# taaha-khan/2023-CompaCT-Image-Compression

Hardware: AMD Instinct MI355X
Metric: MPixels/s encode+decode, 12-bit 512x512 CT batch, bytes-exact (higher is better)
Workload: dtype u16

## Files before the change

2023-compact-image-compression_amd/csrc/deflate_kernels.hip:

```cpp
#include <hip/hip_runtime.h>
#include <cstring>
#include <algorithm>

#include "cct_internal.h"
#include "../../include/compact_hip.h"

namespace cct {
namespace {

constexpr int MIN_MATCH = 3, MAX_MATCH = 258, WSIZE = 32768;
constexpr int MIN_LOOKAHEAD = MAX_MATCH + MIN_MATCH + 1;
constexpr int MAX_DIST = WSIZE - MIN_LOOKAHEAD;
constexpr int TOO_FAR = 4096;
constexpr int BLOCK_SYMS = 16383;
constexpr int BLOCK_SYMS_ML9 = 32767;
constexpr int L_CODES = 286, D_CODES = 30, BL_CODES = 19, HEAP_SIZE = 2 * L_CODES + 1;
constexpr int END_BLOCK = 256, MAX_BITS = 15, MAX_BL_BITS = 7;
constexpr uint32_t Z_FILTERED = 1, Z_HUFFMAN_ONLY = 2, Z_RLE = 3, Z_FIXED = 4;
__host__ __device__ __forceinline__ bool short_pass(uint32_t strategy) { return strategy == Z_HUFFMAN_ONLY || strategy == Z_RLE; }

__constant__ uint8_t c_extra_lbits[29] = {0,0,0,0,0,0,0,0,1,1,1,1,2,2,2,2,3,3,3,3,4,4,4,4,5,5,5,5,0};
__constant__ uint8_t c_extra_dbits[30] = {0,0,0,0,1,1,2,2,3,3,4,4,5,5,6,6,7,7,8,8,9,9,10,10,11,11,12,12,13,13};
__constant__ uint8_t c_extra_blbits[19] = {0,0,0,0,0,0,0,0,0,0,0,0,0,0,0,0,2,3,7};
__constant__ uint8_t c_bl_order[19] = {16,17,18,0,8,7,9,6,10,5,11,4,12,3,13,2,14,1,15};
// ... 1288 lines not shown
				if (R < 4) nlit_head = R;
				else if (R <= 6) { nlit_head = 1; tail_sym = 16u | ((R - 4u) << 5); }
				else {
					nlit_head = 1; nrep6 = 1 + (R - 7u) / 6u;
					const uint32_t r = (R - 7u) % 6u;
					if (r < 3) tail_lit = r; else tail_sym = 16u | ((r - 3u) << 5);
				}
			} else {
				nbig = R / 138u;
				const uint32_t r = R % 138u;
				if (r < 3) tail_lit = r;
				else if (r <= 10) tail_sym = 17u | ((r - 3u) << 5);
				else tail_sym = 18u | ((r - 11u) << 5);
			}
		}
		const uint32_t ntok = nlit_head + nrep6 + nbig + tail_lit + (tail_sym != 0xFFFFFFFFu ? 1u : 0u);
		uint32_t inc = ntok;
#pragma unroll
		for (int d = 1; d < 64; d <<= 1) { const uint32_t o = (uint32_t)__shfl_up((int)inc, d, 64); if (lane >= d) inc += o; }
		if (start) {
			uint32_t w = base + inc - ntok;
			for (uint32_t i = 0; i < nlit_head; i++) tk[w++] = (uint16_t)val;
			for (uint32_t i = 0; i < nrep6; i++) tk[w++] = (uint16_t)(16u | (3u << 5));
			for (uint32_t i = 0; i < nbig; i++) tk[w++] = (uint16_t)(18u | (127u << 5));
			for (uint32_t i = 0; i < tail_lit; i++) tk[w++] = (uint16_t)val;
			if (tail_sym != 0xFFFFFFFFu) tk[w++] = (uint16_t)tail_sym;
			if (nlit_head + tail_lit) atomicAdd(&S.hdr_bits[val], nlit_head + tail_lit);
			if (nrep6) atomicAdd(&S.hdr_bits[16], nrep6);
			if (nbig) atomicAdd(&S.hdr_bits[18], nbig);
			if (tail_sym != 0xFFFFFFFFu) atomicAdd(&S.hdr_bits[tail_sym & 31u], 1u);
		}
		base += (uint32_t)__shfl((int)inc, 63, 64);
	}
	if (lane == 0) S.ntok = (int)base;
}

__device__ __forceinline__ void hdr_or(TreeScratch &S, uint32_t pos, uint32_t value, uint32_t n)
{
	const uint32_t w = pos >> 5, sh = pos & 31u;
	atomicOr(&S.hdr_bits[w], value << sh);
	if (sh + n > 32u) atomicOr(&S.hdr_bits[w + 1], value >> (32u - sh));
}

__device__ void send_header(TreeScratch &S)
{
	const int lane = threadIdx.x;
	const int nbl = S.max_blindex + 1;
	if (lane == 0) hdr_or(S, 0, (uint32_t)(S.lmax + 1 - 257) | ((uint32_t)(S.dmax + 1 - 1) << 5) | ((uint32_t)(nbl - 4) << 10), 14);
	if (lane < nbl) hdr_or(S, 14u + 3u * (uint32_t)lane, S.blen[S.bl_order[lane]], 3);
	uint32_t base = 14u + 3u * (uint32_t)nbl;
	const uint16_t *tk = S.tok();
	const int nt = S.ntok;
	for (int c0 = 0; c0 < nt; c0 += 64) {
		const int i = c0 + lane;
		uint32_t nbits = 0, val = 0;
		if (i < nt) {
			const uint32_t sym = tk[i] & 31u, ex = tk[i] >> 5;
			const uint32_t cl = S.blen[sym];
			nbits = cl + S.extra_bl[sym];
			val = (uint32_t)S.bcode[sym] | (ex << cl);
		}
		uint32_t inc = nbits;
#pragma unroll
		for (int d = 1; d < 64; d <<= 1) { const uint32_t o = (uint32_t)__shfl_up((int)inc, d, 64); if (lane >= d) inc += o; }
		if (nbits) hdr_or(S, base + inc - nbits, val, nbits);
		base += (uint32_t)__shfl((int)inc, 63, 64);
	}
	if (lane == 0) S.hdr_nbits = base;
}

constexpr int TREE_BLOCKS = 1;

__device__ __forceinline__ uint32_t window_base(uint32_t top, uint32_t L, uint32_t strategy)
{
	const uint32_t lam = strategy == Z_HUFFMAN_ONLY ? 0u : strategy == Z_RLE ? (uint32_t)MAX_MATCH : (uint32_t)MIN_LOOKAHEAD - 1u;
	const uint32_t kf = L >= 65536u ? (L - 65536u) / 32768u + 1u : 0u;
	uint32_t k = 0;
	if (top >= 65536u - lam) k = min((top - (65536u - lam)) / 32768u + 1u, kf);
	if (k == kf && 32768u * k + (uint32_t)(WSIZE + MAX_DIST) <= top && L <= top + lam) k++;
	return 32768u * k;
}
__global__ void __launch_bounds__(64) dfl_tree_kernel(DeflateArgs a)
{
	__shared__ TreeScratch S4[TREE_BLOCKS];
	const int s = blockIdx.y, m0 = blockIdx.x * TREE_BLOCKS, lane = threadIdx.x;
	const uint32_t T = a.total_syms[s];
	const uint32_t L = a.in_sizes[s];
	const uint32_t BS = a.block_syms;
	uint32_t nfull = T / BS;
	if (T % BS == 0 && nfull > 0 && !short_pass(a.strategy) && a.postloop_lit[s]) nfull--;
	const uint32_t nblocks = nfull + 1;
	BlockMeta *meta = a.block_meta + (size_t)s * a.max_blocks;
	if ((uint32_t)m0 >= nblocks) return;
	const int nb = (int)min((uint32_t)TREE_BLOCKS, nblocks - (uint32_t)m0);
	const uint32_t *bend = a.blk_end + (size_t)s * a.max_blocks;
	const bool owner = lane < nb;
#ifdef CCT_TREE_PROF
	long long tp[16]; int tpi = 0;
#define TREE_STAMP() do { if (tpi < 16) tp[tpi++] = clock64(); } while (0)
#else
#define TREE_STAMP() do {} while (0)
#endif
	TREE_STAMP();

	for (int q = 0; q < nb; q++) {
		TreeScratch &S = S4[q];
		const int m = m0 + q;
		const bool last = (uint32_t)m == nblocks - 1;
		const uint32_t first = (uint32_t)m * BS;
		const uint32_t nsym = last ? T - first : BS;
		const uint32_t *sym = a.sym + (size_t)s * a.in_stride + first;
		for (int i = lane; i < HEAP_SIZE; i += 64) { S.freq[i] = 0; S.len[i] = 0; }
		for (int i = lane; i < L_CODES + 2; i += 64) S.code[i] = 0;
		for (int i = lane; i < 2 * D_CODES + 1; i += 64) { S.dfreq[i] = 0; S.dlen[i] = 0; S.ddad[i] = 0; }
		for (int i = lane; i < D_CODES + 2; i += 64) S.dcode[i] = 0;
		for (int i = lane; i < 2 * BL_CODES + 1; i += 64) { S.bfreq[i] = 0; S.blen[i] = 0; S.bdad[i] = 0; }
		for (int i = lane; i < BL_CODES + 1; i += 64) S.bcode[i] = 0;
		uint8_t *length_code = S.length_code(), *dist_code = S.dist_code();
		{
			uint8_t dc[8], lc4[4];
#pragma unroll
			for (int k = 0; k < 8; k++) dc[k] = c_dist_code[lane + 64 * k];
#pragma unroll
			for (int k = 0; k < 4; k++) lc4[k] = c_length_code[lane + 64 * k];
			const int l29 = min(lane, 28), l30 = min(lane, 29), l19 = min(lane, 18);
			const uint8_t xl = c_extra_lbits[l29], xd = c_extra_dbits[l30], xb = c_extra_blbits[l19], bo = c_bl_order[l19];
#pragma unroll
			for (int k = 0; k < 8; k++) dist_code[lane + 64 * k] = dc[k];
#pragma unroll
			for (int k = 0; k < 4; k++) length_code[lane + 64 * k] = lc4[k];
			if (lane < 29) S.extra_l[lane] = xl;
			if (lane < 30) S.extra_d[lane] = xd;
			if (lane < 19) { S.extra_bl[lane] = xb; S.bl_order[lane] = bo; }
		}
		uint32_t *hl = S.hist_l(), *hd = S.hist_d();
		for (int i = lane; i < L_CODES; i += 64) hl[i] = 0;
		if (lane < D_CODES) hd[lane] = 0;
		__syncthreads();
		{
			const uint32_t lasts = nsym ? nsym - 1 : 0;
			uint32_t nv[16];
#pragma unroll
			for (int k = 0; k < 16; k++) nv[k] = sym[min((uint32_t)(k * 64 + lane), lasts)];
			for (uint32_t i0 = 0; i0 < nsym; i0 += 64 * 16) {
				uint32_t v[16];
#pragma unroll
				for (int k = 0; k < 16; k++) v[k] = nv[k];
#pragma unroll
				for (int k = 0; k < 16; k++) nv[k] = sym[min(i0 + 1024u + (uint32_t)(k * 64 + lane), lasts)];
#pragma unroll
				for (int k = 0; k < 16; k++) {
					if (i0 + (uint32_t)(k * 64 + lane) >= nsym) continue;
					const uint32_t dist = v[k] >> 16, lc = v[k] & 0xFFu;
					if (dist == 0) atomicAdd(&hl[lc], 1u);
					else {
						const uint32_t d1 = dist - 1;
						atomicAdd(&hl[length_code[lc] + 256 + 1], 1u);
						atomicAdd(&hd[d1 < 256 ? dist_code[d1] : dist_code[256 + (d1 >> 7)]], 1u);
					}
				}
			}
		}
		__syncthreads();
		for (int i = lane; i < L_CODES; i += 64) S.freq[i] = (uint16_t)hl[i];
		if (lane < D_CODES) S.dfreq[lane] = (uint16_t)hd[lane];
		for (int i = lane; i < 160; i += 64) S.hdr_bits[i] = 0;
		if (lane == 0) { S.opt_len = 0; S.static_len = 0; S.hdr_nbits = 0; S.ntok = 0; S.btype = 0; S.max_blindex = 0; }
		__syncthreads();
		if (lane == 0) S.freq[END_BLOCK] = 1;
		for (int i = lane; i < HEAP_SIZE; i += 64) S.dad[i] = 0;
	}
	__syncthreads();
	TREE_STAMP();
#pragma unroll 1
	for (int kind = 0; kind < 3; kind++) {
		if (kind == 2) {
			if (owner) S4[lane].dyn_body_bits = S4[lane].opt_len;
			__syncthreads();
			for (int q = 0; q < nb; q++) {
				TreeScratch &S = S4[q];
				scan_tree_wave(S, view_of(S, 0), S.lmax);
				__syncthreads();
				scan_tree_wave(S, view_of(S, 1), S.dmax);
				__syncthreads();
				if (lane < BL_CODES) { S.bfreq[lane] = (uint16_t)S.hdr_bits[lane]; S.hdr_bits[lane] = 0; }
			}
			__syncthreads();
		}
		for (int q = 0; q < nb; q++) tree_leaves(S4[q], kind);
		__syncthreads();
		TREE_STAMP();
		for (int q = 0; q < nb; q++) tree_heap(S4[q], kind);
		__syncthreads();
		TREE_STAMP();
		for (int q = 0; q < nb; q++) tree_depths(S4[q], kind);
		__syncthreads();
		if (owner) {
			tree_fix(S4[lane], kind);
			if (kind == 0) S4[lane].lmax = S4[lane].max_code; else if (kind == 1) S4[lane].dmax = S4[lane].max_code;
		}
		__syncthreads();
		for (int q = 0; q < nb; q++) tree_codes(S4[q], kind);
		__syncthreads();
		TREE_STAMP();
	}
	if (owner) {
		TreeScratch &S = S4[lane];
		const int m = m0 + lane;
		const bool last = (uint32_t)m == nblocks - 1;
		const uint32_t first = (uint32_t)m * BS;
		const uint32_t nsym = last ? T - first : BS;
		const uint32_t in_begin = m == 0 ? 0u : bend[m - 1];
		const uint32_t in_end = last ? L : bend[m];
		int max_blindex;
		for (max_blindex = BL_CODES - 1; max_blindex >= 3; max_blindex--)
			if (S.blen[S.bl_order[max_blindex]] != 0) break;
		S.opt_len += 3 * ((uint32_t)max_blindex + 1) + 5 + 5 + 4;
		uint32_t opt_lenb = (S.opt_len + 3 + 7) >> 3;
		const uint32_t static_lenb = (S.static_len + 3 + 7) >> 3;
		if (static_lenb <= opt_lenb) opt_lenb = static_lenb;
		const uint32_t stored_len = in_end - in_begin;
		const bool in_window = in_begin >= window_base(last ? L : a.blk_top[(size_t)s * a.max_blocks + m], L, a.strategy);
		BlockMeta bm;
		bm.in_begin = in_begin; bm.stored_len = stored_len; bm.first_sym = first; bm.nsym = nsym; bm.last = last ? 1u : 0u;
		if (in_window && stored_len + 4 <= opt_lenb) {
			bm.type = 0; bm.hdr_nbits = 0; bm.body_bits = 0;
		} else if (a.strategy == Z_FIXED || static_lenb == opt_lenb) {
			bm.type = 1; bm.hdr_nbits = 0; bm.body_bits = S.static_len;
		} else {
			bm.type = 2; bm.hdr_nbits = 0;
			bm.body_bits = S.dyn_body_bits;
		}
		S.btype = (int)bm.type; S.max_blindex = max_blindex;
		meta[m] = bm;
		if (m == 0) a.n_blocks[s] = nblocks;
	}
	__syncthreads();
	for (int q = 0; q < nb; q++) {
		TreeScratch &S = S4[q];
		if (S.btype != 2) continue;
		send_header(S);
		__syncthreads();
		BlockTables *bt = a.block_tables + ((size_t)s * a.max_blocks + m0 + q);
		for (int i = lane; i * 32 < (int)S.hdr_nbits; i += 64) bt->hdr_bits[i] = S.hdr_bits[i];
		if (lane == 0) meta[m0 + q].hdr_nbits = S.hdr_nbits;
	}
	__syncthreads();
	TREE_STAMP();
#ifdef CCT_TREE_PROF
	if (s == 0 && m0 == 0 && lane == 0) {
		printf("[tree prof] nb=%d:", nb);
		for (int i = 1; i < tpi; i++) printf(" %lld", tp[i] - tp[i - 1]);
		printf("  (hist | leaves0 heap0 rest0 | scan+leaves1 heap1 rest1 | scan_tree+leaves2 heap2 rest2 | final)\n");
	}
#endif
	for (int q = 0; q < nb; q++) {
		TreeScratch &S = S4[q];
		BlockTables *bt = a.block_tables + ((size_t)s * a.max_blocks + m0 + q);
		for (int i = lane; i < L_CODES; i += 64) { bt->lcode[i] = S.code[i]; bt->llen[i] = (uint8_t)S.len[i]; }
		if (lane < D_CODES) { bt->dcode[lane] = S.dcode[lane]; bt->dlen[lane] = (uint8_t)S.dlen[lane]; }
	}
}

__global__ void __launch_bounds__(256) dfl_adler_kernel(DeflateArgs a)
{
	__shared__ unsigned long long sa[256], sb[256];
	const int s = blockIdx.x;
	const uint32_t L = a.in_sizes[s];
	const uint8_t *in = a.in + (size_t)s * a.in_stride;
	unsigned long long A = 0, B = 0;
	const uint32_t nfull = L / 16;
	constexpr int U = 8;
	for (uint32_t g0 = threadIdx.x; g0 < nfull; g0 += blockDim.x * U) {
		uint4 v[U];
#pragma unroll
		for (int u = 0; u < U; u++) v[u] = *reinterpret_cast<const uint4 *>(in + (size_t)min(g0 + (uint32_t)u * blockDim.x, nfull - 1) * 16);
#pragma unroll
		for (int u = 0; u < U; u++) {
			const uint32_t g = g0 + (uint32_t)u * blockDim.x;
			if (g >= nfull) continue;
			const uint32_t w[4] = {v[u].x, v[u].y, v[u].z, v[u].w};
			uint32_t sd = 0, sk = 0;
#pragma unroll
			for (int k = 0; k < 16; k++) { const uint32_t d = (w[k >> 2] >> ((k & 3) * 8)) & 0xFFu; sd += d; sk += (uint32_t)k * d; }
			A += sd;
			B += (unsigned long long)(L - g * 16) * sd - sk;
		}
	}
	if (threadIdx.x == 0)
		for (uint32_t i = nfull * 16; i < L; i++) { const unsigned long long d = in[i]; A += d; B += (unsigned long long)(L - i) * d; }
	sa[threadIdx.x] = A; sb[threadIdx.x] = B;
	__syncthreads();
	for (int st = 128; st > 0; st >>= 1) {
		if ((int)threadIdx.x < st) { sa[threadIdx.x] += sa[threadIdx.x + st]; sb[threadIdx.x] += sb[threadIdx.x + st]; }
		__syncthreads();
	}
	if (threadIdx.x == 0) {
		const uint32_t lo = (uint32_t)((1ull + sa[0]) % 65521ull);
		const uint32_t hi = (uint32_t)(((unsigned long long)L + sb[0]) % 65521ull);
		a.adler[s] = (hi << 16) | lo;
	}
}

__global__ void dfl_layout_kernel(DeflateArgs a, int n)
{
	const int s = blockIdx.x * blockDim.x + threadIdx.x;
	if (s >= n) return;
	uint8_t *out = a.out + (size_t)s * a.out_stride;
	for (int i = 0; i < 13; i++) out[i] = a.header13[i];
	out[13] = 0x78; out[14] = (uint8_t)a.zlib_flg;
	uint64_t bit = 8ull * 15;
	BlockMeta *meta = a.block_meta + (size_t)s * a.max_blocks;
	const uint32_t nb = a.n_blocks[s];
	for (uint32_t m = 0; m < nb; m++) {
		BlockMeta bm = meta[m];
		bm.bit_off = bit;
		if (bm.type == 0) {
			bit = (bit + 3 + 7) & ~7ull;
			bit += 32 + 8ull * bm.stored_len;
		} else {
			bit += 3 + bm.hdr_nbits + bm.body_bits;
		}
		if (bm.last) bit = (bit + 7) & ~7ull;
		meta[m] = bm;
	}
	const uint64_t byte = bit >> 3;
	const uint32_t ad = a.adler[s];
	out[byte + 0] = (uint8_t)(ad >> 24); out[byte + 1] = (uint8_t)(ad >> 16);
	out[byte + 2] = (uint8_t)(ad >> 8);  out[byte + 3] = (uint8_t)ad;
	a.out_sizes[s] = (uint32_t)(byte + 4);
}

__device__ __forceinline__ void or_bits(uint32_t *words, uint64_t bit, uint64_t value, int nbits)
{
	if (nbits == 0) return;
	const uint64_t w = bit >> 5;
	const int sh = (int)(bit & 31);
	const uint64_t lo = value << sh;
	const uint64_t hi = sh ? (value >> (64 - sh)) : 0ull;
	atomicOr(&words[w], (uint32_t)lo);
	if (sh + nbits > 32) atomicOr(&words[w + 1], (uint32_t)(lo >> 32));
	if (sh + nbits > 64) atomicOr(&words[w + 2], (uint32_t)hi);
}

__global__ void __launch_bounds__(256) dfl_emit_kernel(DeflateArgs a)
{
	__shared__ uint32_t wsum[4];
	__shared__ unsigned long long s_run;
	const int s = blockIdx.y, m = blockIdx.x;
	if ((uint32_t)m >= a.n_blocks[s]) return;
	const BlockMeta bm = a.block_meta[(size_t)s * a.max_blocks + m];
	const BlockTables *bt = a.block_tables + ((size_t)s * a.max_blocks + m);
	uint8_t *out = a.out + (size_t)s * a.out_stride;
	uint32_t *words = reinterpret_cast<uint32_t *>(out);
	const uint8_t *in = a.in + (size_t)s * a.in_stride;
	uint64_t bit = bm.bit_off;
	if (bm.type == 0) {
		if (threadIdx.x == 0) or_bits(words, bit, (uint64_t)bm.last, 3);
		const uint64_t byte = ((bit + 3 + 7) & ~7ull) >> 3;
		if (threadIdx.x == 0) {
			out[byte] = (uint8_t)(bm.stored_len & 0xFF); out[byte + 1] = (uint8_t)(bm.stored_len >> 8);
			out[byte + 2] = (uint8_t)(~bm.stored_len & 0xFF); out[byte + 3] = (uint8_t)((~bm.stored_len >> 8) & 0xFF);
		}
		for (uint32_t i = threadIdx.x; i < bm.stored_len; i += blockDim.x) out[byte + 4 + i] = in[bm.in_begin + i];
		return;
	}
	if (threadIdx.x == 0) or_bits(words, bit, (uint64_t)((bm.type << 1) + bm.last), 3);
	bit += 3;
	if (bm.type == 2) {
		for (uint32_t i = threadIdx.x; i * 32 < bm.hdr_nbits; i += blockDim.x) {
			const int nb = (int)min(32u, bm.hdr_nbits - i * 32);
			or_bits(words, bit + 32ull * i, bt->hdr_bits[i], nb);
		}
		bit += bm.hdr_nbits;
	}
	const uint32_t *sym = a.sym + (size_t)s * a.in_stride + bm.first_sym;
	const bool dyn = bm.type == 2;
	const int lane = threadIdx.x & 63, wave = threadIdx.x >> 6;
	__shared__ uint16_t t_lcode[L_CODES + 2], t_dcode[D_CODES + 2];
	__shared__ uint8_t t_llen[L_CODES + 2], t_dlen[D_CODES + 2];
	__shared__ uint32_t wbuf[400];
	__shared__ uint8_t t_length_code[256], t_dist_code[512], t_extra_l[32], t_extra_d[32];
	__shared__ uint16_t t_base_length[32], t_base_dist[32];
	{
		const int t = threadIdx.x, t2 = min(t + 256, L_CODES - 1), td = min(t, D_CODES - 1), t29 = min(t, 28), t30 = min(t, 29);
		const uint16_t *lsrc = dyn ? bt->lcode : c_static_lcode, *dsrc = dyn ? bt->dcode : c_static_dcode;
		const uint8_t *llsrc = dyn ? bt->llen : c_static_llen;
		const uint16_t lc0 = lsrc[t], lc1 = lsrc[t2];
		const uint8_t ll0 = llsrc[t], ll1 = llsrc[t2];
		const uint16_t dc = dsrc[td];
		uint8_t dl = bt->dlen[td];
		if (!dyn) dl = 5;
		const uint8_t k0 = c_dist_code[t], k1 = c_dist_code[t + 256], lcd = c_length_code[t];
		const uint8_t xl = c_extra_lbits[t29], xd = c_extra_dbits[t30];
		const uint16_t bl = c_base_length[t29], bd = c_base_dist[t30];
		t_lcode[t] = lc0; t_llen[t] = ll0;
		if (t + 256 < L_CODES) { t_lcode[t + 256] = lc1; t_llen[t + 256] = ll1; }
		if (t < D_CODES) { t_dcode[t] = dc; t_dlen[t] = dl; }
		t_dist_code[t] = k0; t_dist_code[t + 256] = k1; t_length_code[t] = lcd;
		if (t < 29) { t_extra_l[t] = xl; t_base_length[t] = bl; }
		if (t < 30) { t_extra_d[t] = xd; t_base_dist[t] = bd; }
	}
	if (threadIdx.x == 0) s_run = bit;
	for (int i = threadIdx.x; i < 400; i += blockDim.x) wbuf[i] = 0;
	__syncthreads();
	const uint32_t last_sym = bm.nsym ? bm.nsym - 1 : 0;
	uint32_t vnext = sym[min((uint32_t)threadIdx.x, last_sym)];
	for (uint32_t base = 0; base <= bm.nsym; base += blockDim.x) {
		const uint32_t i = base + threadIdx.x;
		uint64_t bits = 0;
		int nb = 0;
		const uint32_t v = vnext;
		vnext = sym[min(i + blockDim.x, last_sym)];
		if (i < bm.nsym) {
			uint32_t dist = v >> 16;
			const uint32_t lc = v & 0xFFu;
			if (dist == 0) {
				bits = t_lcode[lc];
				nb = t_llen[lc];
			} else {
				int code = t_length_code[lc];
				const int lsym = code + 256 + 1;
				bits = t_lcode[lsym];
				nb = t_llen[lsym];
				int extra = t_extra_l[code];
				if (extra) { bits |= (uint64_t)(lc - t_base_length[code]) << nb; nb += extra; }
				dist--;
				code = dist < 256 ? t_dist_code[dist] : t_dist_code[256 + (dist >> 7)];
				bits |= (uint64_t)t_dcode[code] << nb;
				nb += t_dlen[code];
				extra = t_extra_d[code];
				if (extra) { bits |= (uint64_t)(dist - t_base_dist[code]) << nb; nb += extra; }
			}
		} else if (i == bm.nsym) {
			bits = t_lcode[END_BLOCK];
			nb = t_llen[END_BLOCK];
		}
		uint32_t inc = (uint32_t)nb;
#pragma unroll
		for (int d = 1; d < 64; d <<= 1) {
			const uint32_t t = __shfl_up(inc, d);
			if (lane >= d) inc += t;
		}
		if (lane == 63) wsum[wave] = inc;
		__syncthreads();
		uint32_t wb = 0, tot = 0;
		for (int w = 0; w < 4; w++) { if (w < wave) wb += wsum[w]; tot += wsum[w]; }
		const uint64_t run = s_run;
		const uint32_t lbit = (uint32_t)(run & 31) + wb + inc - (uint32_t)nb;
		if (nb) {
			const uint32_t w0 = lbit >> 5, sh = lbit & 31;
			const uint64_t lo = bits << sh;
			atomicOr(&wbuf[w0], (uint32_t)lo);
			if (sh + nb > 32) atomicOr(&wbuf[w0 + 1], (uint32_t)(lo >> 32));
			if (sh + nb > 64) atomicOr(&wbuf[w0 + 2], (uint32_t)(bits >> (64 - sh)));
		}
		__syncthreads();
		const uint32_t nwords = ((uint32_t)(run & 31) + tot + 31) >> 5;
		const uint64_t gw = run >> 5;
		for (uint32_t k = threadIdx.x; k < nwords; k += blockDim.x) {
			const uint32_t v = wbuf[k];
			if (v) atomicOr(&words[gw + k], v);
			wbuf[k] = 0;
		}
		if (threadIdx.x == 0) s_run = run + tot;
		__syncthreads();
	}
}

__global__ void __launch_bounds__(256) dfl_pack_offsets_kernel(const uint32_t *sizes, int n, uint64_t *offsets, int exact)
{
	if (threadIdx.x == 0 && blockIdx.x == 0) {
		uint64_t acc = 0;
		for (int i = 0; i < n; i++) { offsets[i] = acc; acc += exact ? sizes[i] : ((sizes[i] + 15u) & ~15u); }
		offsets[n] = acc;
	}
}
__global__ void __launch_bounds__(256) dfl_pack_kernel(const uint8_t *src, size_t stride, const uint32_t *sizes,
                                                       const uint64_t *offsets, uint8_t *dst)
{
	const int s = blockIdx.y;
	const uint32_t n16 = (sizes[s] + 15u) >> 4;
	const uint4 *in = reinterpret_cast<const uint4 *>(src + (size_t)s * stride);
	uint4 *out = reinterpret_cast<uint4 *>(dst + offsets[s]);
	for (uint32_t i = blockIdx.x * blockDim.x + threadIdx.x; i < n16; i += gridDim.x * blockDim.x) out[i] = in[i];
}

__global__ void dfl_offsets2_kernel(DeflateArgs a, int n)
{
	const size_t per = a.in_stride / 64;
	for (size_t i = blockIdx.x * (size_t)blockDim.x + threadIdx.x; i < (size_t)n * per; i += (size_t)gridDim.x * blockDim.x)
		a.blk_entry[i] = 0xFFFFFFFFu;
}

__global__ void dfl_offsets_kernel(DeflateArgs a, int n)
{
	if (blockIdx.x == 0) {
		for (int s = threadIdx.x; s < n; s += blockDim.x) { a.postloop_lit[s] = 0; a.heavy_count[s] = 0; a.deep_count[s] = 0; a.run_end_count[s] = 0; }
		if (threadIdx.x == 0) *a.gen = *a.gen % GEN_MAX + 1u;
	}
	const size_t nrc = (size_t)n * 2 * (size_t)a.run_chunks;
	for (size_t t = (size_t)blockIdx.x * blockDim.x + threadIdx.x; t < nrc; t += (size_t)gridDim.x * blockDim.x) a.run_counts[t] = 0;
}

}

bool deflate_level_args(int level, DeflateArgs &a)
{
	static const uint32_t T[6][5] = {
		{4, 4, 16, 16, 0x5E}, {8, 16, 32, 32, 0x5E}, {8, 16, 128, 128, 0x9C},
		{8, 32, 128, 256, 0xDA}, {32, 128, 258, 1024, 0xDA}, {32, 258, 258, 4096, 0xDA},
	};
	if (level < 4 || level > 9) return false;
	const uint32_t *t = T[level - 4];
	a.good = t[0]; a.max_lazy = t[1]; a.nice = t[2]; a.max_chain = t[3]; a.zlib_flg = t[4];
	return true;
}

bool deflate_strategy_args(int level, int strategy, DeflateArgs &a)
{
	if (strategy < 0 || strategy > (int)Z_FIXED) return false;
	a.strategy = (uint32_t)strategy;
	a.min_len = strategy == (int)Z_FILTERED ? 6u : (uint32_t)MIN_MATCH;
	if (short_pass((uint32_t)strategy)) {
		if (level < 1 || level > 9) return false;
		a.good = a.max_lazy = a.nice = a.max_chain = 0;
		a.zlib_flg = 0x01;
		return true;
	}
	if (!deflate_level_args(level, a)) return false;
	if (strategy == (int)Z_FIXED) a.zlib_flg = 0x01;
	return true;
}

bool deflate_mem_level_args(int mem_level, DeflateArgs &a)
{
	if (mem_level != 8 && mem_level != 9) return false;
	a.hash_bits = (uint32_t)mem_level + 7u;
	a.block_syms = (1u << (mem_level + 6)) - 1u;
	return true;
}

hipError_t deflate_init_tables()
{
	uint8_t length_code[256]; uint16_t base_length[29]; uint8_t dist_code[512]; uint16_t base_dist[30];
	uint16_t static_lcode[288]; uint8_t static_llen[288]; uint16_t static_dcode[30];
	static const int xl[29] = {0,0,0,0,0,0,0,0,1,1,1,1,2,2,2,2,3,3,3,3,4,4,4,4,5,5,5,5,0};
	static const int xd[30] = {0,0,0,0,1,1,2,2,3,3,4,4,5,5,6,6,7,7,8,8,9,9,10,10,11,11,12,12,13,13};
	int length = 0, code, n, dist = 0;
	for (code = 0; code < 28; code++) {
		base_length[code] = (uint16_t)length;
		for (n = 0; n < (1 << xl[code]); n++) length_code[length++] = (uint8_t)code;
	}
	length_code[length - 1] = (uint8_t)code;
	base_length[28] = 0;
	for (code = 0; code < 16; code++) {
		base_dist[code] = (uint16_t)dist;
		for (n = 0; n < (1 << xd[code]); n++) dist_code[dist++] = (uint8_t)code;
	}
	dist >>= 7;
	for (; code < 30; code++) {
		base_dist[code] = (uint16_t)(dist << 7);
		for (n = 0; n < (1 << (xd[code] - 7)); n++) dist_code[256 + dist++] = (uint8_t)code;
	}
	uint16_t bl_count[16] = {0}, next_code[16];
	n = 0;
	while (n <= 143) { static_llen[n++] = 8; bl_count[8]++; }
	while (n <= 255) { static_llen[n++] = 9; bl_count[9]++; }
	while (n <= 279) { static_llen[n++] = 7; bl_count[7]++; }
	while (n <= 287) { static_llen[n++] = 8; bl_count[8]++; }
	unsigned c = 0;
	for (int bits = 1; bits <= 15; bits++) { c = (c + bl_count[bits - 1]) << 1; next_code[bits] = (uint16_t)c; }
	auto rev = [](unsigned v, int len) { unsigned r = 0; do { r |= v & 1; v >>= 1; r <<= 1; } while (--len > 0); return r >> 1; };
	for (n = 0; n < 288; n++) static_lcode[n] = (uint16_t)rev(next_code[static_llen[n]]++, static_llen[n]);
	for (n = 0; n < 30; n++) static_dcode[n] = (uint16_t)rev((unsigned)n, 5);
	hipError_t e;
	if ((e = hipMemcpyToSymbol(HIP_SYMBOL(c_length_code), length_code, sizeof length_code)) != hipSuccess) return e;
	if ((e = hipMemcpyToSymbol(HIP_SYMBOL(c_base_length), base_length, sizeof base_length)) != hipSuccess) return e;
	if ((e = hipMemcpyToSymbol(HIP_SYMBOL(c_dist_code), dist_code, sizeof dist_code)) != hipSuccess) return e;
	if ((e = hipMemcpyToSymbol(HIP_SYMBOL(c_base_dist), base_dist, sizeof base_dist)) != hipSuccess) return e;
	if ((e = hipMemcpyToSymbol(HIP_SYMBOL(c_static_lcode), static_lcode, sizeof static_lcode)) != hipSuccess) return e;
	if ((e = hipMemcpyToSymbol(HIP_SYMBOL(c_static_llen), static_llen, sizeof static_llen)) != hipSuccess) return e;
	if ((e = hipMemcpyToSymbol(HIP_SYMBOL(c_static_dcode), static_dcode, sizeof static_dcode)) != hipSuccess) return e;
	return hipSuccess;
}

size_t deflate_sort_temp_bytes(size_t total, int n)
{
	(void)total; (void)n;
	return 0;
}

static hipError_t launch_deflate_short(const DeflateArgs &a, int n, hipStream_t st)
{
	const bool ml9 = a.block_syms == (uint32_t)BLOCK_SYMS_ML9;
	const int gx = (int)std::min<size_t>(64, (a.in_stride + 255) / 256);
	if (a.strategy == Z_RLE) {
		hipLaunchKernelGGL((dfl_run_len_kernel<false, 15>), dim3(gx, n), dim3(256), 0, st, a);
		hipLaunchKernelGGL(dfl_rle_rec_kernel, dim3(gx, n), dim3(256), 0, st, a);
		hipLaunchKernelGGL(dfl_offsets2_kernel, dim3(256), dim3(256), 0, st, a, n);
		hipLaunchKernelGGL(dfl_walk_kernel, dim3(n), dim3(WALK_T), 0, st, a, n);
		if (ml9) hipLaunchKernelGGL(dfl_symbols_kernel<BLOCK_SYMS_ML9>, dim3(gx, n), dim3(256), 0, st, a);
		else hipLaunchKernelGGL(dfl_symbols_kernel<BLOCK_SYMS>, dim3(gx, n), dim3(256), 0, st, a);
	} else {
		if (ml9) hipLaunchKernelGGL(dfl_huff_symbols_kernel<BLOCK_SYMS_ML9>, dim3(gx, n), dim3(256), 0, st, a);
		else hipLaunchKernelGGL(dfl_huff_symbols_kernel<BLOCK_SYMS>, dim3(gx, n), dim3(256), 0, st, a);
	}
	hipLaunchKernelGGL(dfl_adler_kernel, dim3(n), dim3(256), 0, st, a);
	hipLaunchKernelGGL(dfl_tree_kernel, dim3((a.max_blocks + TREE_BLOCKS - 1) / TREE_BLOCKS, n), dim3(64), 0, st, a);
	hipLaunchKernelGGL(dfl_layout_kernel, dim3((n + 63) / 64), dim3(64), 0, st, a, n);
	hipLaunchKernelGGL(dfl_emit_kernel, dim3(a.max_blocks, n), dim3(256), 0, st, a);
	return hipGetLastError();
}

hipError_t launch_deflate(const DeflateArgs &a, int n, void *sort_temp, size_t sort_temp_bytes, hipStream_t st, hipStream_t side,
                          const hipEvent_t *ev)
{
	hipError_t e;
	const bool ml9 = a.hash_bits == 16;
	if ((a.hash_bits != 15 && !ml9) || a.block_syms != (uint32_t)(ml9 ? BLOCK_SYMS_ML9 : BLOCK_SYMS)) return hipErrorInvalidValue;
	if (ml9 && a.pos_mask != 0xFFFFFFFFu) return hipErrorInvalidValue;
	if ((e = hipMemsetAsync(a.out, 0, (size_t)n * a.out_stride, st)) != hipSuccess) return e;
	if (short_pass(a.strategy)) return launch_deflate_short(a, n, st);
	if ((e = hipMemsetAsync(a.sort_hist, 0, (size_t)n * SORT_HIST * 4, st)) != hipSuccess) return e;
	hipLaunchKernelGGL(dfl_offsets_kernel, dim3(64), dim3(256), 0, st, a, n);
	const int gx = (int)std::min<size_t>(64, (a.in_stride + 255) / 256);
	(void)sort_temp; (void)sort_temp_bytes;
	if (ml9) {
		hipLaunchKernelGGL((dfl_run_len_kernel<true, 16>), dim3(gx, n), dim3(256), 0, st, a);
		hipLaunchKernelGGL((dfl_sort_pass_kernel<true, 16>), dim3(n), dim3(1024), 0, st, a);
		hipLaunchKernelGGL((dfl_sort_pass_kernel<false, 16>), dim3(n), dim3(1024), 0, st, a);
	} else {
		hipLaunchKernelGGL((dfl_run_len_kernel<true, 15>), dim3(gx, n), dim3(256), 0, st, a);
		hipLaunchKernelGGL((dfl_sort_pass_kernel<true, 15>), dim3(n), dim3(1024), 0, st, a);
		hipLaunchKernelGGL((dfl_sort_pass_kernel<false, 15>), dim3(n), dim3(1024), 0, st, a);
	}
	const bool fork = side != nullptr && ev != nullptr;
	hipStream_t s2 = fork ? side : st;
	if (fork) {
		if ((e = hipEventRecord(ev[0], st)) != hipSuccess) return e;
		if ((e = hipStreamWaitEvent(s2, ev[0], 0)) != hipSuccess) return e;
	}
	hipLaunchKernelGGL(dfl_run_lists_kernel, dim3(a.run_chunks, n), dim3(256), 0, s2, a);
	hipLaunchKernelGGL(dfl_run_info_kernel, dim3(8, n), dim3(256), 0, s2, a);
	const int gm_cap = a.pos_mask == COMPACT_POS_MASK ? 256 : 2048;
	const int gm = (int)std::min<size_t>(gm_cap, (a.in_stride + 255) / 256), n8 = (n + 7) & ~7;
	if (a.max_chain < 16 || a.max_chain > 4096 || a.nice < 16 || a.nice > (uint32_t)MAX_MATCH) return hipErrorInvalidValue;
	const bool ql = (a.max_chain >> 2) <= (uint32_t)LIGHT_STEPS;
	if (a.pos_mask == COMPACT_POS_MASK) {
		if (ql) hipLaunchKernelGGL((dfl_match_kernel<true, true>), dim3(gm, n8), dim3(256), 0, st, a, n);
		else hipLaunchKernelGGL((dfl_match_kernel<true, false>), dim3(gm, n8), dim3(256), 0, st, a, n);
	} else if (a.pos_mask == 0xFFFFFFFFu) {
		if (ql) hipLaunchKernelGGL((dfl_match_kernel<false, true>), dim3(gm, n8), dim3(256), 0, st, a, n);
		else hipLaunchKernelGGL((dfl_match_kernel<false, false>), dim3(gm, n8), dim3(256), 0, st, a, n);
	} else return hipErrorInvalidValue;
	if (fork) {
		if ((e = hipEventRecord(ev[1], st)) != hipSuccess) return e;
		if ((e = hipEventRecord(ev[2], s2)) != hipSuccess) return e;
		if ((e = hipStreamWaitEvent(s2, ev[1], 0)) != hipSuccess) return e;
		if ((e = hipStreamWaitEvent(st, ev[2], 0)) != hipSuccess) return e;
	}
	hipLaunchKernelGGL(dfl_match_heavy_kernel, dim3(gx, n8), dim3(256), 0, s2, a, n);
	hipLaunchKernelGGL(dfl_adler_kernel, dim3(n), dim3(256), 0, s2, a);
	hipLaunchKernelGGL(dfl_match_run_kernel, dim3(gx, n8), dim3(256), 0, st, a, n);
	if (fork) {
		if ((e = hipEventRecord(ev[3], s2)) != hipSuccess) return e;
		if ((e = hipStreamWaitEvent(st, ev[3], 0)) != hipSuccess) return e;
	}
	hipLaunchKernelGGL(dfl_rec_kernel, dim3(gx, n), dim3(256), 0, st, a);
	hipLaunchKernelGGL(dfl_offsets2_kernel, dim3(256), dim3(256), 0, st, a, n);
	hipLaunchKernelGGL(dfl_walk_kernel, dim3(n), dim3(WALK_T), 0, st, a, n);
	if (ml9) hipLaunchKernelGGL(dfl_symbols_kernel<BLOCK_SYMS_ML9>, dim3(gx, n), dim3(256), 0, st, a);
	else hipLaunchKernelGGL(dfl_symbols_kernel<BLOCK_SYMS>, dim3(gx, n), dim3(256), 0, st, a);
	hipLaunchKernelGGL(dfl_tree_kernel, dim3((a.max_blocks + TREE_BLOCKS - 1) / TREE_BLOCKS, n), dim3(64), 0, st, a);
	hipLaunchKernelGGL(dfl_layout_kernel, dim3((n + 63) / 64), dim3(64), 0, st, a, n);
	hipLaunchKernelGGL(dfl_emit_kernel, dim3(a.max_blocks, n), dim3(256), 0, st, a);
	return hipGetLastError();
}

__global__ void __launch_bounds__(256) dfl_pack_exact_kernel(const uint8_t *src, size_t stride, const uint32_t *sizes,
                                                             const uint64_t *offsets, uint8_t *dst)
{
	const int s = blockIdx.y;
	const uint32_t nbytes = sizes[s];
	const uint8_t *in = src + (size_t)s * stride;
	uint8_t *out = dst + offsets[s];
	for (uint32_t i = blockIdx.x * blockDim.x + threadIdx.x; i < nbytes; i += gridDim.x * blockDim.x) out[i] = in[i];
}

hipError_t launch_pack(const uint8_t *src, size_t stride, const uint32_t *sizes, int n, uint64_t *offsets, uint8_t *dst,
                       int exact, hipStream_t st)
{
	hipLaunchKernelGGL(dfl_pack_offsets_kernel, dim3(1), dim3(64), 0, st, sizes, n, offsets, exact);
	if (exact) hipLaunchKernelGGL(dfl_pack_exact_kernel, dim3(32, n), dim3(256), 0, st, src, stride, sizes, offsets, dst);
	else hipLaunchKernelGGL(dfl_pack_kernel, dim3(16, n), dim3(256), 0, st, src, stride, sizes, offsets, dst);
	return hipGetLastError();
}

}
```

Before: 16100.

## Parallelize layout, pack offsets, multi-symbol emit, and replace memsets with bounded clears

The layout kernel now gives one wavefront per stream and passes block sizes between lanes with shuffles, and the pack-offsets kernel becomes a block-wide scan instead of a serial loop. The emit kernel now has each thread encode several symbols into local limbs, and double-buffers its shared word buffer so one barrier per iteration goes away. Its interior words are written with plain stores instead of atomics. Full-buffer memsets are replaced by a clear kernel that zeroes only the bounded output size, runs on the side stream, and also clears the sort histogram. The exact pack copy uses 32-bit words with shift alignment, and offsets2 is moved onto the side stream.

```diff
diff --git a/2023-compact-image-compression_amd/csrc/deflate_kernels.hip b/2023-compact-image-compression_amd/csrc/deflate_kernels.hip
--- a/2023-compact-image-compression_amd/csrc/deflate_kernels.hip
+++ b/2023-compact-image-compression_amd/csrc/deflate_kernels.hip
@@ -1614,33 +1614,38 @@
 	}
 }
 
-__global__ void dfl_layout_kernel(DeflateArgs a, int n)
-{
-	const int s = blockIdx.x * blockDim.x + threadIdx.x;
+__global__ void __launch_bounds__(64) dfl_layout_kernel(DeflateArgs a, int n)
+{
+	const int s = blockIdx.x, lane = threadIdx.x;
 	if (s >= n) return;
 	uint8_t *out = a.out + (size_t)s * a.out_stride;
-	for (int i = 0; i < 13; i++) out[i] = a.header13[i];
-	out[13] = 0x78; out[14] = (uint8_t)a.zlib_flg;
-	uint64_t bit = 8ull * 15;
 	BlockMeta *meta = a.block_meta + (size_t)s * a.max_blocks;
 	const uint32_t nb = a.n_blocks[s];
-	for (uint32_t m = 0; m < nb; m++) {
-		BlockMeta bm = meta[m];
-		bm.bit_off = bit;
-		if (bm.type == 0) {
-			bit = (bit + 3 + 7) & ~7ull;
-			bit += 32 + 8ull * bm.stored_len;
-		} else {
-			bit += 3 + bm.hdr_nbits + bm.body_bits;
-		}
-		if (bm.last) bit = (bit + 7) & ~7ull;
-		meta[m] = bm;
-	}
-	const uint64_t byte = bit >> 3;
 	const uint32_t ad = a.adler[s];
-	out[byte + 0] = (uint8_t)(ad >> 24); out[byte + 1] = (uint8_t)(ad >> 16);
-	out[byte + 2] = (uint8_t)(ad >> 8);  out[byte + 3] = (uint8_t)ad;
-	a.out_sizes[s] = (uint32_t)(byte + 4);
+	uint64_t bit = 8ull * 15;
+	for (uint32_t m0 = 0; m0 < nb; m0 += 64) {
+		const uint32_t m = m0 + (uint32_t)lane, cnt = min(64u, nb - m0);
+		const BlockMeta bm = meta[min(m, nb - 1)];
+		const uint32_t flags = (bm.type == 0 ? 1u : 0u) | (bm.last ? 2u : 0u);
+		const uint64_t size = bm.type == 0 ? 32 + 8ull * bm.stored_len : 3ull + bm.hdr_nbits + bm.body_bits;
+		uint64_t mine = 0;
+		for (uint32_t j = 0; j < cnt; j++) {
+			const uint32_t fj = __shfl(flags, (int)j);
+			const uint64_t zj = __shfl((unsigned long long)size, (int)j);
+			if (j == (uint32_t)lane) mine = bit;
+			bit = (fj & 1u) ? ((bit + 3 + 7) & ~7ull) + zj : bit + zj;
+			if (fj & 2u) bit = (bit + 7) & ~7ull;
+		}
+		if (m < nb) meta[m].bit_off = mine;
+	}
+	if (lane == 0) {
+		for (int i = 0; i < 13; i++) out[i] = a.header13[i];
+		out[13] = 0x78; out[14] = (uint8_t)a.zlib_flg;
+		const uint64_t byte = bit >> 3;
+		out[byte + 0] = (uint8_t)(ad >> 24); out[byte + 1] = (uint8_t)(ad >> 16);
+		out[byte + 2] = (uint8_t)(ad >> 8);  out[byte + 3] = (uint8_t)ad;
+		a.out_sizes[s] = (uint32_t)(byte + 4);
+	}
 }
 
 __device__ __forceinline__ void or_bits(uint32_t *words, uint64_t bit, uint64_t value, int nbits)
@@ -1655,10 +1660,16 @@
 	if (sh + nbits > 64) atomicOr(&words[w + 2], (uint32_t)hi);
 }
 
+#ifndef CCT_EMIT_K
+#define CCT_EMIT_K 4
+#endif
+constexpr int EMIT_K = CCT_EMIT_K;
+constexpr int EMIT_T = 256 * EMIT_K;
+constexpr int EMIT_LIMBS = (EMIT_K * 48 + 63) / 64;
+constexpr int EMIT_WBUF = EMIT_T * 48 / 32 + 8;
 __global__ void __launch_bounds__(256) dfl_emit_kernel(DeflateArgs a)
 {
-	__shared__ uint32_t wsum[4];
-	__shared__ unsigned long long s_run;
+	__shared__ uint32_t wsum[2][4];
 	const int s = blockIdx.y, m = blockIdx.x;
 	if ((uint32_t)m >= a.n_blocks[s]) return;
 	const BlockMeta bm = a.block_meta[(size_t)s * a.max_blocks + m];
@@ -1691,7 +1702,7 @@
 	const int lane = threadIdx.x & 63, wave = threadIdx.x >> 6;
 	__shared__ uint16_t t_lcode[L_CODES + 2], t_dcode[D_CODES + 2];
 	__shared__ uint8_t t_llen[L_CODES + 2], t_dlen[D_CODES + 2];
-	__shared__ uint32_t wbuf[400];
+	__shared__ uint32_t wbuf[2][EMIT_WBUF];
 	__shared__ uint8_t t_length_code[256], t_dist_code[512], t_extra_l[32], t_extra_d[32];
 	__shared__ uint16_t t_base_length[32], t_base_dist[32];
 	{
@@ -1713,80 +1724,122 @@
 		if (t < 29) { t_extra_l[t] = xl; t_base_length[t] = bl; }
 		if (t < 30) { t_extra_d[t] = xd; t_base_dist[t] = bd; }
 	}
-	if (threadIdx.x == 0) s_run = bit;
-	for (int i = threadIdx.x; i < 400; i += blockDim.x) wbuf[i] = 0;
+	for (int i = threadIdx.x; i < 2 * EMIT_WBUF; i += blockDim.x) (&wbuf[0][0])[i] = 0;
 	__syncthreads();
 	const uint32_t last_sym = bm.nsym ? bm.nsym - 1 : 0;
-	uint32_t vnext = sym[min((uint32_t)threadIdx.x, last_sym)];
-	for (uint32_t base = 0; base <= bm.nsym; base += blockDim.x) {
-		const uint32_t i = base + threadIdx.x;
-		uint64_t bits = 0;
-		int nb = 0;
-		const uint32_t v = vnext;
-		vnext = sym[min(i + blockDim.x, last_sym)];
-		if (i < bm.nsym) {
-			uint32_t dist = v >> 16;
-			const uint32_t lc = v & 0xFFu;
-			if (dist == 0) {
-				bits = t_lcode[lc];
-				nb = t_llen[lc];
-			} else {
-				int code = t_length_code[lc];
-				const int lsym = code + 256 + 1;
-				bits = t_lcode[lsym];
-				nb = t_llen[lsym];
-				int extra = t_extra_l[code];
-				if (extra) { bits |= (uint64_t)(lc - t_base_length[code]) << nb; nb += extra; }
-				dist--;
-				code = dist < 256 ? t_dist_code[dist] : t_dist_code[256 + (dist >> 7)];
-				bits |= (uint64_t)t_dcode[code] << nb;
-				nb += t_dlen[code];
-				extra = t_extra_d[code];
-				if (extra) { bits |= (uint64_t)(dist - t_base_dist[code]) << nb; nb += extra; }
-			}
-		} else if (i == bm.nsym) {
-			bits = t_lcode[END_BLOCK];
-			nb = t_llen[END_BLOCK];
-		}
-		uint32_t inc = (uint32_t)nb;
+	uint32_t vnext[EMIT_K];
+#pragma unroll
+	for (int k = 0; k < EMIT_K; k++) vnext[k] = sym[min((uint32_t)(threadIdx.x * EMIT_K + k), last_sym)];
+	uint64_t run = bit;
+	int par = 0;
+	for (uint32_t base = 0; base <= bm.nsym; base += EMIT_T, par ^= 1) {
+		const uint32_t i0 = base + threadIdx.x * EMIT_K;
+		uint32_t v[EMIT_K];
+#pragma unroll
+		for (int k = 0; k < EMIT_K; k++) v[k] = vnext[k];
+#pragma unroll
+		for (int k = 0; k < EMIT_K; k++) vnext[k] = sym[min(i0 + (uint32_t)(EMIT_T + k), last_sym)];
+		uint64_t acc[EMIT_LIMBS];
+#pragma unroll
+		for (int j = 0; j < EMIT_LIMBS; j++) acc[j] = 0;
+		uint32_t ltot = 0;
+#pragma unroll
+		for (int k = 0; k < EMIT_K; k++) {
+			const uint32_t i = i0 + k;
+			uint64_t bits = 0;
+			int nb = 0;
+			if (i < bm.nsym) {
+				uint32_t dist = v[k] >> 16;
+				const uint32_t lc = v[k] & 0xFFu;
+				if (dist == 0) {
+					bits = t_lcode[lc];
+					nb = t_llen[lc];
+				} else {
+					int code = t_length_code[lc];
+					const int lsym = code + 256 + 1;
+					bits = t_lcode[lsym];
+					nb = t_llen[lsym];
+					int extra = t_extra_l[code];
+					if (extra) { bits |= (uint64_t)(lc - t_base_length[code]) << nb; nb += extra; }
+					dist--;
+					code = dist < 256 ? t_dist_code[dist] : t_dist_code[256 + (dist >> 7)];
+					bits |= (uint64_t)t_dcode[code] << nb;
+					nb += t_dlen[code];
+					extra = t_extra_d[code];
+					if (extra) { bits |= (uint64_t)(dist - t_base_dist[code]) << nb; nb += extra; }
+				}
+			} else if (i == bm.nsym) {
+				bits = t_lcode[END_BLOCK];
+				nb = t_llen[END_BLOCK];
+			}
+			const uint32_t q = ltot >> 6, r = ltot & 63;
+			const uint64_t lo = bits << r, hi = r ? bits >> (64 - r) : 0ull;
+#pragma unroll
+			for (int j = 0; j < EMIT_LIMBS; j++) {
+				if (q == (uint32_t)j) acc[j] |= lo;
+				if (q + 1 == (uint32_t)j) acc[j] |= hi;
+			}
+			ltot += (uint32_t)nb;
+		}
+		uint32_t inc = ltot;
 #pragma unroll
 		for (int d = 1; d < 64; d <<= 1) {
 			const uint32_t t = __shfl_up(inc, d);
 			if (lane >= d) inc += t;
 		}
-		if (lane == 63) wsum[wave] = inc;
+		if (lane == 63) wsum[par][wave] = inc;
 		__syncthreads();
 		uint32_t wb = 0, tot = 0;
-		for (int w = 0; w < 4; w++) { if (w < wave) wb += wsum[w]; tot += wsum[w]; }
-		const uint64_t run = s_run;
-		const uint32_t lbit = (uint32_t)(run & 31) + wb + inc - (uint32_t)nb;
-		if (nb) {
-			const uint32_t w0 = lbit >> 5, sh = lbit & 31;
-			const uint64_t lo = bits << sh;
-			atomicOr(&wbuf[w0], (uint32_t)lo);
-			if (sh + nb > 32) atomicOr(&wbuf[w0 + 1], (uint32_t)(lo >> 32));
-			if (sh + nb > 64) atomicOr(&wbuf[w0 + 2], (uint32_t)(bits >> (64 - sh)));
+		for (int w = 0; w < 4; w++) { if (w < wave) wb += wsum[par][w]; tot += wsum[par][w]; }
+		uint32_t *wbf = wbuf[par];
+		const uint32_t lbit = (uint32_t)(run & 31) + wb + inc - ltot;
+		if (ltot) {
+			const uint32_t w0 = lbit >> 5, sh = lbit & 31, nw = (sh + ltot + 31) >> 5;
+#pragma unroll
+			for (int j = 0; j <= 2 * EMIT_LIMBS; j++) {
+				const uint32_t aj = j < 2 * EMIT_LIMBS ? (uint32_t)(acc[j >> 1] >> (32 * (j & 1))) : 0u;
+				const uint32_t ap = j > 0 ? (uint32_t)(acc[(j - 1) >> 1] >> (32 * ((j - 1) & 1))) : 0u;
+				const uint32_t w = (uint32_t)((((uint64_t)aj << 32) | ap) >> (32 - sh));
+				if ((uint32_t)j < nw && w) atomicOr(&wbf[w0 + j], w);
+			}
 		}
 		__syncthreads();
 		const uint32_t nwords = ((uint32_t)(run & 31) + tot + 31) >> 5;
 		const uint64_t gw = run >> 5;
 		for (uint32_t k = threadIdx.x; k < nwords; k += blockDim.x) {
-			const uint32_t v = wbuf[k];
-			if (v) atomicOr(&words[gw + k], v);
-			wbuf[k] = 0;
-		}
-		if (threadIdx.x == 0) s_run = run + tot;
+			const uint32_t w = wbf[k];
+			wbf[k] = 0;
+			if (k == 0 || k == nwords - 1) { if (w) atomicOr(&words[gw + k], w); }
+			else words[gw + k] = w;
+		}
+		run += tot;
+	}
+}
+
+__global__ void __launch_bounds__(256) dfl_pack_offsets_kernel(const uint32_t *sizes, int n, uint64_t *offsets, int exact)
+{
+	__shared__ unsigned long long wsum[4];
+	const int t = threadIdx.x, lane = t & 63, wave = t >> 6;
+	unsigned long long carry = 0;
+	for (int base = 0; base < n; base += 256) {
+		const int i = base + t;
+		const uint32_t sz = i < n ? sizes[i] : 0u;
+		const unsigned long long v = exact ? sz : (unsigned long long)((sz + 15u) & ~15u);
+		unsigned long long inc = v;
+#pragma unroll
+		for (int d = 1; d < 64; d <<= 1) {
+			const unsigned long long u = __shfl_up(inc, d);
+			if (lane >= d) inc += u;
+		}
+		if (lane == 63) wsum[wave] = inc;
 		__syncthreads();
-	}
-}
-
-__global__ void __launch_bounds__(256) dfl_pack_offsets_kernel(const uint32_t *sizes, int n, uint64_t *offsets, int exact)
-{
-	if (threadIdx.x == 0 && blockIdx.x == 0) {
-		uint64_t acc = 0;
-		for (int i = 0; i < n; i++) { offsets[i] = acc; acc += exact ? sizes[i] : ((sizes[i] + 15u) & ~15u); }
-		offsets[n] = acc;
-	}
+		unsigned long long wb = 0, tot = 0;
+		for (int w = 0; w < 4; w++) { if (w < wave) wb += wsum[w]; tot += wsum[w]; }
+		if (i < n) offsets[i] = carry + wb + inc - v;
+		carry += tot;
+		__syncthreads();
+	}
+	if (t == 0) offsets[n] = carry;
 }
 __global__ void __launch_bounds__(256) dfl_pack_kernel(const uint8_t *src, size_t stride, const uint32_t *sizes,
                                                        const uint64_t *offsets, uint8_t *dst)
@@ -1811,8 +1864,31 @@
 		for (int s = threadIdx.x; s < n; s += blockDim.x) { a.postloop_lit[s] = 0; a.heavy_count[s] = 0; a.deep_count[s] = 0; a.run_end_count[s] = 0; }
 		if (threadIdx.x == 0) *a.gen = *a.gen % GEN_MAX + 1u;
 	}
-	const size_t nrc = (size_t)n * 2 * (size_t)a.run_chunks;
-	for (size_t t = (size_t)blockIdx.x * blockDim.x + threadIdx.x; t < nrc; t += (size_t)gridDim.x * blockDim.x) a.run_counts[t] = 0;
+	const size_t nrc = (size_t)n * (SORT_HIST + 2 * (size_t)a.run_chunks);
+	for (size_t t = (size_t)blockIdx.x * blockDim.x + threadIdx.x; t < nrc; t += (size_t)gridDim.x * blockDim.x) a.sort_hist[t] = 0;
+}
+
+constexpr uint32_t CLEAR_SLACK = 64;
+__device__ __forceinline__ size_t clear_bytes(const DeflateArgs &a, int s)
+{
+	const size_t L = a.in_sizes[s];
+	const size_t bound = a.block_syms == (uint32_t)BLOCK_SYMS ? L + (L >> 12) + (L >> 14) + (L >> 25) + 13
+	                                                          : L + ((L + 7) >> 3) + ((L + 63) >> 6) + 5 + 6;
+	return min(a.out_stride, (13 + bound + CLEAR_SLACK + 15) & ~(size_t)15);
+}
+template <typename W>
+__global__ void __launch_bounds__(256) dfl_clear_kernel(DeflateArgs a)
+{
+	const int s = blockIdx.y;
+	const size_t units = clear_bytes(a, s) / sizeof(W);
+	W *out = reinterpret_cast<W *>(a.out + (size_t)s * a.out_stride);
+	W zero{};
+	for (size_t i = blockIdx.x * (size_t)blockDim.x + threadIdx.x; i < units; i += (size_t)gridDim.x * blockDim.x) out[i] = zero;
+}
+static void launch_clear(const DeflateArgs &a, int n, hipStream_t st)
+{
+	if (a.out_stride % 16 == 0 && (uintptr_t)a.out % 16 == 0) hipLaunchKernelGGL(dfl_clear_kernel<uint4>, dim3(16, n), dim3(256), 0, st, a);
+	else hipLaunchKernelGGL(dfl_clear_kernel<uint32_t>, dim3(32, n), dim3(256), 0, st, a);
 }
 
 }
@@ -1907,6 +1983,7 @@
 {
 	const bool ml9 = a.block_syms == (uint32_t)BLOCK_SYMS_ML9;
 	const int gx = (int)std::min<size_t>(64, (a.in_stride + 255) / 256);
+	launch_clear(a, n, st);
 	if (a.strategy == Z_RLE) {
 		hipLaunchKernelGGL((dfl_run_len_kernel<false, 15>), dim3(gx, n), dim3(256), 0, st, a);
 		hipLaunchKernelGGL(dfl_rle_rec_kernel, dim3(gx, n), dim3(256), 0, st, a);
@@ -1920,7 +1997,7 @@
 	}
 	hipLaunchKernelGGL(dfl_adler_kernel, dim3(n), dim3(256), 0, st, a);
 	hipLaunchKernelGGL(dfl_tree_kernel, dim3((a.max_blocks + TREE_BLOCKS - 1) / TREE_BLOCKS, n), dim3(64), 0, st, a);
-	hipLaunchKernelGGL(dfl_layout_kernel, dim3((n + 63) / 64), dim3(64), 0, st, a, n);
+	hipLaunchKernelGGL(dfl_layout_kernel, dim3(n), dim3(64), 0, st, a, n);
 	hipLaunchKernelGGL(dfl_emit_kernel, dim3(a.max_blocks, n), dim3(256), 0, st, a);
 	return hipGetLastError();
 }
@@ -1932,9 +2009,8 @@
 	const bool ml9 = a.hash_bits == 16;
 	if ((a.hash_bits != 15 && !ml9) || a.block_syms != (uint32_t)(ml9 ? BLOCK_SYMS_ML9 : BLOCK_SYMS)) return hipErrorInvalidValue;
 	if (ml9 && a.pos_mask != 0xFFFFFFFFu) return hipErrorInvalidValue;
-	if ((e = hipMemsetAsync(a.out, 0, (size_t)n * a.out_stride, st)) != hipSuccess) return e;
+	if ((a.out_stride & 3) || ((uintptr_t)a.out & 3)) return hipErrorInvalidValue;
 	if (short_pass(a.strategy)) return launch_deflate_short(a, n, st);
-	if ((e = hipMemsetAsync(a.sort_hist, 0, (size_t)n * SORT_HIST * 4, st)) != hipSuccess) return e;
 	hipLaunchKernelGGL(dfl_offsets_kernel, dim3(64), dim3(256), 0, st, a, n);
 	const int gx = (int)std::min<size_t>(64, (a.in_stride + 255) / 256);
 	(void)sort_temp; (void)sort_temp_bytes;
@@ -1955,6 +2031,8 @@
 	}
 	hipLaunchKernelGGL(dfl_run_lists_kernel, dim3(a.run_chunks, n), dim3(256), 0, s2, a);
 	hipLaunchKernelGGL(dfl_run_info_kernel, dim3(8, n), dim3(256), 0, s2, a);
+	launch_clear(a, n, s2);
+	hipLaunchKernelGGL(dfl_offsets2_kernel, dim3(256), dim3(256), 0, s2, a, n);
 	const int gm_cap = a.pos_mask == COMPACT_POS_MASK ? 256 : 2048;
 	const int gm = (int)std::min<size_t>(gm_cap, (a.in_stride + 255) / 256), n8 = (n + 7) & ~7;
 	if (a.max_chain < 16 || a.max_chain > 4096 || a.nice < 16 || a.nice > (uint32_t)MAX_MATCH) return hipErrorInvalidValue;
@@ -1980,12 +2058,11 @@
 		if ((e = hipStreamWaitEvent(st, ev[3], 0)) != hipSuccess) return e;
 	}
 	hipLaunchKernelGGL(dfl_rec_kernel, dim3(gx, n), dim3(256), 0, st, a);
-	hipLaunchKernelGGL(dfl_offsets2_kernel, dim3(256), dim3(256), 0, st, a, n);
 	hipLaunchKernelGGL(dfl_walk_kernel, dim3(n), dim3(WALK_T), 0, st, a, n);
 	if (ml9) hipLaunchKernelGGL(dfl_symbols_kernel<BLOCK_SYMS_ML9>, dim3(gx, n), dim3(256), 0, st, a);
 	else hipLaunchKernelGGL(dfl_symbols_kernel<BLOCK_SYMS>, dim3(gx, n), dim3(256), 0, st, a);
 	hipLaunchKernelGGL(dfl_tree_kernel, dim3((a.max_blocks + TREE_BLOCKS - 1) / TREE_BLOCKS, n), dim3(64), 0, st, a);
-	hipLaunchKernelGGL(dfl_layout_kernel, dim3((n + 63) / 64), dim3(64), 0, st, a, n);
+	hipLaunchKernelGGL(dfl_layout_kernel, dim3(n), dim3(64), 0, st, a, n);
 	hipLaunchKernelGGL(dfl_emit_kernel, dim3(a.max_blocks, n), dim3(256), 0, st, a);
 	return hipGetLastError();
 }
@@ -1997,13 +2074,25 @@
 	const uint32_t nbytes = sizes[s];
 	const uint8_t *in = src + (size_t)s * stride;
 	uint8_t *out = dst + offsets[s];
-	for (uint32_t i = blockIdx.x * blockDim.x + threadIdx.x; i < nbytes; i += gridDim.x * blockDim.x) out[i] = in[i];
+	const uint32_t head = min((uint32_t)(-(uintptr_t)out & 3u), nbytes);
+	const uint32_t nd = (nbytes - head) >> 2;
+	const uint32_t tid = blockIdx.x * blockDim.x + threadIdx.x, nth = gridDim.x * blockDim.x;
+	const uint32_t *in32 = reinterpret_cast<const uint32_t *>(in);
+	uint32_t *out32 = reinterpret_cast<uint32_t *>(out + head);
+	const uint32_t sh = 8u * head, up = head ? 1u : 0u;
+	for (uint32_t j = tid; j < nd; j += nth) {
+		const uint64_t pair = ((uint64_t)in32[j + up] << 32) | in32[j];
+		out32[j] = (uint32_t)(pair >> sh);
+	}
+	const uint32_t tail0 = head + 4u * nd;
+	if (tid < head) out[tid] = in[tid];
+	if (tid < nbytes - tail0) out[tail0 + tid] = in[tail0 + tid];
 }
 
 hipError_t launch_pack(const uint8_t *src, size_t stride, const uint32_t *sizes, int n, uint64_t *offsets, uint8_t *dst,
                        int exact, hipStream_t st)
 {
-	hipLaunchKernelGGL(dfl_pack_offsets_kernel, dim3(1), dim3(64), 0, st, sizes, n, offsets, exact);
+	hipLaunchKernelGGL(dfl_pack_offsets_kernel, dim3(1), dim3(256), 0, st, sizes, n, offsets, exact);
 	if (exact) hipLaunchKernelGGL(dfl_pack_exact_kernel, dim3(32, n), dim3(256), 0, st, src, stride, sizes, offsets, dst);
 	else hipLaunchKernelGGL(dfl_pack_kernel, dim3(16, n), dim3(256), 0, st, src, stride, sizes, offsets, dst);
 	return hipGetLastError();
```

Result: faster. 16630 (median of 6 runs) (+3.3%).
